# Angel3245/p2pfl

Measured on AMD Instinct MI355X. Metric: train samples/s (aggregate over peers); wall-clock per FedAvg round in ms_per_step, higher is better.
Workload: dtype bf16; 1 GPU; model=MNIST-CNN (p2pfl CNN: conv5x5 32/64 + FC 3136-2048-10, 6.5M params), Adam 1e-3, global_batch=32, per_peer_round=2700 train + 300 val + 500 test samples, 1 epoch, parallelism=gossip-p2p

## Files before the change

### csrc/cnn.h

```cpp
#pragma once
#include <hip/hip_runtime.h>
#include <stdint.h>

namespace p2cnn {

constexpr int kImg = 28;
constexpr int kC1 = 32;
constexpr int kC2 = 64;
constexpr int kFeat = 3136;
constexpr int kHid = 2048;
constexpr int kCls = 10;
constexpr int kTaps = 25;
constexpr int kXcdSplits = 7;
bool xcd_align();

struct AdamCfg {
  float lr, beta1, beta2, eps, weight_decay;
};

struct Offsets {
  int64_t c1w, c1b, c2w, c2b, l1w, l1b, l2w, l2b;
};

void conv1_fwd(const uint8_t* x, const int64_t* idx, const float* params, Offsets off, uint16_t* p1, uint8_t* am1,
// ... 7 lines not shown

void gemm_skinny(const uint16_t* A, const uint16_t* Bt, float* slabs, int mrows, int N, int K, int S, hipStream_t s);

void head(const float* slabs, int S, int mrows, const float* params, Offsets off, const int64_t* labels,
          const int64_t* idx, int B, int train, uint16_t* H, uint16_t* dH, float* dlogits, float* stats,
          const uint16_t* w2bf, hipStream_t s);

void fc1_wgrad_adam(const uint16_t* dH, const uint16_t* a1, int mrows, float* params, float* m, float* v,
                    float* gdump, uint16_t* w1bf, uint16_t* w1tbf, Offsets off, const int* adam_t, int t_off,
                    AdamCfg cfg, hipStream_t s);

void route_fc2(const uint16_t* dH, const uint16_t* w1t, const uint8_t* am2, int mrows, int B, uint16_t* dc2m,
               float* gb, const float* dlogits, const uint16_t* H, float* params, float* m, float* v, float* gdump,
               Offsets off, const int* adam_t, int t_off, AdamCfg cfg, bool with_fc2, hipStream_t s);

void route_fc2_rm(const uint16_t* dH, const uint16_t* w1, const uint8_t* am2, int mrows, int B, uint16_t* dc2m,
                  float* gb, const float* dlogits, const uint16_t* H, float* params, float* m, float* v,
                  float* gdump, Offsets off, const int* adam_t, int t_off, AdamCfg cfg, bool with_fc2,
                  float* ws, int* ctr, hipStream_t s);

void conv2_bwd(const uint16_t* dc2m, const uint16_t* p1s, const uint8_t* am1, const uint16_t* w2q, const uint8_t* x,
               const int64_t* idx, float* wslab1, float* wslab2, int B, hipStream_t s);

void conv_adam(const float* wslab1, const float* wslab2, const float* gb, int B, float* params, float* m, float* v,
               float* gdump, uint16_t* w2r, uint16_t* w2q, Offsets off, const int* adam_t, int t_off, AdamCfg cfg,
               hipStream_t s);

struct FwdNext {
  const uint8_t* x;
  const int64_t* idx;
  uint16_t* p1;
  uint8_t* am1;
  uint16_t* p1s;
  uint16_t* a1;
  uint8_t* am2;
  int B;
  int* sync;
};
void fc1_conv_adam_fwd(const uint16_t* dH, const uint16_t* a1, int mrows, const float* wslab1, const float* wslab2,
                       const float* gb, int B, float* params, float* m, float* v, float* gdump, uint16_t* w1bf,
                       uint16_t* w1tbf, uint16_t* w2r, uint16_t* w2q, Offsets off, const int* adam_t, int t_off,
                       AdamCfg cfg, const float* dlogits, const uint16_t* H, uint16_t* w2bf, const FwdNext& f,
                       hipStream_t s);

void fc1_conv_adam(const uint16_t* dH, const uint16_t* a1, int mrows, const float* wslab1, const float* wslab2,
                   const float* gb, int B, float* params, float* m, float* v, float* gdump, uint16_t* w1bf,
                   uint16_t* w1tbf, uint16_t* w2r, uint16_t* w2q, Offsets off, const int* adam_t, int t_off,
                   AdamCfg cfg, const float* dlogits, const uint16_t* H, uint16_t* w2bf, hipStream_t s);

void pack_shadows(const float* params, Offsets off, uint16_t* w2r, uint16_t* w2q, uint16_t* w1bf, uint16_t* w1tbf,
                  uint16_t* w2bf, hipStream_t s);

constexpr int kP1sPlane = 18 * 16;
constexpr int kP1s = 5 * kC1 * kP1sPlane;
constexpr int kDgTiles = 7;
constexpr int kSlab1 = kC1 * kTaps + kC1;
constexpr int kWgG = 2;
constexpr int kSlab2 = kTaps * kC2 * kC1;
__host__ __device__ inline int wgrad_groups(int B) { return (B + kWgG - 1) / kWgG; }

}
```

### csrc/cnn_bindings.cpp

```cpp
#include <torch/extension.h>
#include <c10/hip/HIPStream.h>
#include <c10/core/DeviceGuard.h>

#include "cnn.h"

namespace {

using p2cnn::AdamCfg;
using p2cnn::Offsets;

hipStream_t stream() { return c10::hip::getCurrentHIPStream().stream(); }

template <typename T>
T* ptr(const torch::Tensor& t, c10::ScalarType st, int64_t min_numel, const char* name, int align = 16) {
  TORCH_CHECK(t.defined() && t.is_cuda(), name, ": expected a GPU tensor");
  TORCH_CHECK(t.scalar_type() == st, name, ": wrong dtype ", t.scalar_type());
  TORCH_CHECK(t.is_contiguous(), name, ": must be contiguous");
  TORCH_CHECK(t.numel() >= min_numel, name, ": needs >= ", min_numel, " elements, got ", t.numel());
  TORCH_CHECK(reinterpret_cast<uintptr_t>(t.data_ptr()) % align == 0, name, ": must be ", align, "-byte aligned");
  return reinterpret_cast<T*>(t.data_ptr());
}
template <typename T>
T* optr(const c10::optional<torch::Tensor>& t, c10::ScalarType st, int64_t min_numel, const char* name,
        int align = 16) {
// ... 133 lines not shown
  const auto dHp = reinterpret_cast<uint16_t*>(ptr<at::BFloat16>(dH, torch::kBFloat16, mrows * 2048, "dH"));
  const auto w1p = reinterpret_cast<uint16_t*>(ptr<at::BFloat16>(w1, torch::kBFloat16, 2048 * 3136, "w1"));
  const auto am2p = ptr<uint8_t>(am2, torch::kUInt8, B * 3136, "am2");
  const auto dc2p = reinterpret_cast<uint16_t*>(ptr<at::BFloat16>(dc2m, torch::kBFloat16, B * 64 * 224, "dc2m"));
  const auto gbp = ptr<float>(gb, torch::kFloat32, B * 3136, "gb");
  const auto dlp = ptr<float>(dlogits, torch::kFloat32, B * 10, "dlogits");
  const auto Hp = reinterpret_cast<uint16_t*>(ptr<at::BFloat16>(H, torch::kBFloat16, B * 2048, "H"));
  float* pp = ptr<float>(params, torch::kFloat32, n, "params");
  float* mp = ptr<float>(m, torch::kFloat32, n, "m");
  float* vp = ptr<float>(v, torch::kFloat32, n, "v");
  float* gd = optr<float>(gdump, torch::kFloat32, n, "gdump");
  const int* tp = ptr<int>(adam_t, torch::kInt32, 1, "adam_t", 4);
  if (row_major) {
    float* wsp = optr<float>(ws, torch::kFloat32, 98 * 2 * mrows * 32, "ws");
    int* cp = optr<int>(ctr, torch::kInt32, 98, "ctr", 4);
    p2cnn::route_fc2_rm(dHp, w1p, am2p, int(mrows), int(B), dc2p, gbp, dlp, Hp, pp, mp, vp, gd, o, tp, int(t_off),
                        cfg(lr, b1, b2, eps, wd), with_fc2, wsp, cp, stream());
  } else {
    p2cnn::route_fc2(dHp, w1p, am2p, int(mrows), int(B), dc2p, gbp, dlp, Hp, pp, mp, vp, gd, o, tp, int(t_off),
                     cfg(lr, b1, b2, eps, wd), with_fc2, stream());
  }
}

void k_conv2_bwd(torch::Tensor dc2m, torch::Tensor p1s, torch::Tensor am1, torch::Tensor w2q, torch::Tensor x,
                 c10::optional<torch::Tensor> idx, torch::Tensor wslab1, torch::Tensor wslab2, int64_t B) {
  const c10::DeviceGuard g(dc2m.device());
  TORCH_CHECK(B >= 1 && B <= 64, "bad batch");
  TORCH_CHECK(x.numel() % 784 == 0, "x must be [N,1,28,28] uint8");
  if (!idx.has_value()) TORCH_CHECK(x.numel() / 784 >= B, "x has fewer than B rows");
  p2cnn::conv2_bwd(reinterpret_cast<uint16_t*>(ptr<at::BFloat16>(dc2m, torch::kBFloat16, B * 64 * 224, "dc2m")),
                   reinterpret_cast<uint16_t*>(ptr<at::BFloat16>(p1s, torch::kBFloat16, B * p2cnn::kP1s, "p1s")),
                   ptr<uint8_t>(am1, torch::kUInt8, B * 196 * 32, "am1"),
                   reinterpret_cast<uint16_t*>(ptr<at::BFloat16>(w2q, torch::kBFloat16, 51200, "w2q")),
                   ptr<uint8_t>(x, torch::kUInt8, 784, "x", 1), idx_ptr(idx, B),
                   ptr<float>(wslab1, torch::kFloat32, B * p2cnn::kDgTiles * p2cnn::kSlab1, "wslab1"),
                   ptr<float>(wslab2, torch::kFloat32, p2cnn::wgrad_groups(int(B)) * int64_t(p2cnn::kSlab2), "wslab2"),
                   int(B), stream());
}

void k_conv_adam(torch::Tensor wslab1, torch::Tensor wslab2, torch::Tensor gb, int64_t B, torch::Tensor params,
                 torch::Tensor m,
                 torch::Tensor v, c10::optional<torch::Tensor> gdump, torch::Tensor w2r, torch::Tensor w2q,
                 std::vector<int64_t> off, torch::Tensor adam_t, int64_t t_off, double lr, double b1, double b2,
                 double eps, double wd) {
  const c10::DeviceGuard g(params.device());
  Offsets o = offsets(off);
  const int64_t n = params_end(o);
  TORCH_CHECK(B >= 1 && B <= 64, "bad batch");
  p2cnn::conv_adam(ptr<float>(wslab1, torch::kFloat32, B * p2cnn::kDgTiles * p2cnn::kSlab1, "wslab1"),
                   ptr<float>(wslab2, torch::kFloat32, p2cnn::wgrad_groups(int(B)) * int64_t(p2cnn::kSlab2), "wslab2"),
                   ptr<float>(gb, torch::kFloat32, B * 3136, "gb"), int(B),
                   ptr<float>(params, torch::kFloat32, n, "params"), ptr<float>(m, torch::kFloat32, n, "m"),
                   ptr<float>(v, torch::kFloat32, n, "v"), optr<float>(gdump, torch::kFloat32, n, "gdump"),
                   reinterpret_cast<uint16_t*>(ptr<at::BFloat16>(w2r, torch::kBFloat16, 51200, "w2r")),
                   reinterpret_cast<uint16_t*>(ptr<at::BFloat16>(w2q, torch::kBFloat16, 51200, "w2q")), o,
                   ptr<int>(adam_t, torch::kInt32, 1, "adam_t", 4), int(t_off), cfg(lr, b1, b2, eps, wd), stream());
}

void k_fc1_conv_adam(torch::Tensor dH, torch::Tensor a1, int64_t mrows, torch::Tensor wslab1, torch::Tensor wslab2,
                     torch::Tensor gb, int64_t B, torch::Tensor params, torch::Tensor m, torch::Tensor v,
                     c10::optional<torch::Tensor> gdump, torch::Tensor w1bf, c10::optional<torch::Tensor> w1tbf, torch::Tensor w2r,
                     torch::Tensor w2q, std::vector<int64_t> off, torch::Tensor adam_t, int64_t t_off, double lr,
                     double b1, double b2, double eps, double wd, c10::optional<torch::Tensor> dlogits,
                     c10::optional<torch::Tensor> H, c10::optional<torch::Tensor> w2bf) {
  const c10::DeviceGuard g(params.device());
  check_batch(int(B), int(mrows));
  TORCH_CHECK(mrows <= 64, "fc1_conv_adam: mrows must be 32 or 64");
  TORCH_CHECK(dlogits.has_value() == H.has_value(), "fc1_conv_adam: pass both dlogits and H or neither");
  Offsets o = offsets(off);
  const int64_t n = params_end(o);
  p2cnn::fc1_conv_adam(
      reinterpret_cast<uint16_t*>(ptr<at::BFloat16>(dH, torch::kBFloat16, mrows * 2048, "dH")),
      reinterpret_cast<uint16_t*>(ptr<at::BFloat16>(a1, torch::kBFloat16, mrows * 3136, "a1")), int(mrows),
      ptr<float>(wslab1, torch::kFloat32, B * p2cnn::kDgTiles * p2cnn::kSlab1, "wslab1"),
      ptr<float>(wslab2, torch::kFloat32, p2cnn::wgrad_groups(int(B)) * int64_t(p2cnn::kSlab2), "wslab2"),
      ptr<float>(gb, torch::kFloat32, B * 3136, "gb"), int(B), ptr<float>(params, torch::kFloat32, n, "params"),
      ptr<float>(m, torch::kFloat32, n, "m"), ptr<float>(v, torch::kFloat32, n, "v"),
      optr<float>(gdump, torch::kFloat32, n, "gdump"),
      reinterpret_cast<uint16_t*>(ptr<at::BFloat16>(w1bf, torch::kBFloat16, 2048 * 3136, "w1bf")),
      reinterpret_cast<uint16_t*>(optr<at::BFloat16>(w1tbf, torch::kBFloat16, 2048 * 3136, "w1tbf")),
      reinterpret_cast<uint16_t*>(ptr<at::BFloat16>(w2r, torch::kBFloat16, 51200, "w2r")),
      reinterpret_cast<uint16_t*>(ptr<at::BFloat16>(w2q, torch::kBFloat16, 51200, "w2q")), o,
      ptr<int>(adam_t, torch::kInt32, 1, "adam_t", 4), int(t_off), cfg(lr, b1, b2, eps, wd),
      optr<float>(dlogits, torch::kFloat32, B * 10, "dlogits"),
      reinterpret_cast<const uint16_t*>(optr<at::BFloat16>(H, torch::kBFloat16, B * 2048, "H")),
      reinterpret_cast<uint16_t*>(optr<at::BFloat16>(w2bf, torch::kBFloat16, 10 * 2048, "w2bf")), stream());
}

void k_fc1_conv_adam_fwd(torch::Tensor dH, torch::Tensor a1, int64_t mrows, torch::Tensor wslab1, torch::Tensor wslab2,
                         torch::Tensor gb, int64_t B, torch::Tensor params, torch::Tensor m, torch::Tensor v,
                         c10::optional<torch::Tensor> gdump, torch::Tensor w1bf, c10::optional<torch::Tensor> w1tbf,
                         torch::Tensor w2r, torch::Tensor w2q, std::vector<int64_t> off, torch::Tensor adam_t,
                         int64_t t_off, double lr, double b1, double b2, double eps, double wd,
                         c10::optional<torch::Tensor> dlogits, c10::optional<torch::Tensor> H,
                         c10::optional<torch::Tensor> w2bf, torch::Tensor x, c10::optional<torch::Tensor> idx,
                         torch::Tensor p1, torch::Tensor am1, torch::Tensor p1s, torch::Tensor a1n, torch::Tensor am2,
                         int64_t Bn, torch::Tensor sync) {
  const c10::DeviceGuard g(params.device());
  check_batch(int(B), int(mrows));
  check_batch(int(Bn), int(mrows));
  TORCH_CHECK(mrows <= 64, "fc1_conv_adam_fwd: mrows must be 32 or 64");
  TORCH_CHECK(dlogits.has_value() == H.has_value(), "fc1_conv_adam_fwd: pass both dlogits and H or neither");
  TORCH_CHECK(x.numel() % 784 == 0, "x must be [N,1,28,28] uint8");
  if (!idx.has_value()) TORCH_CHECK(x.numel() / 784 >= Bn, "x has fewer than Bn rows");
  TORCH_CHECK(a1n.data_ptr() != a1.data_ptr(), "fc1_conv_adam_fwd: the next step's A1 must be the other buffer");
  Offsets o = offsets(off);
  const int64_t n = params_end(o);
  p2cnn::FwdNext f{};
  f.x = ptr<uint8_t>(x, torch::kUInt8, 784, "x", 1);
// ... 40 lines not shown

namespace p2cnn {
void init_attributes();
}

void register_cnn(pybind11::module& m) {
  auto c = m.def_submodule("cnn", "fused MNIST-CNN training step kernels");
  c.def("init", &p2cnn::init_attributes, "set kernel attributes (call before HIP graph capture)");
  c.def("conv1_fwd", &k_conv1_fwd);
  c.def("conv2_fwd", &k_conv2_fwd);
  c.def("conv12_fwd", &k_conv12_fwd);
  c.def("gemm_skinny", &k_gemm_skinny);
  c.def("head", &k_head, pybind11::arg("slabs"), pybind11::arg("S"), pybind11::arg("mrows"), pybind11::arg("params"),
        pybind11::arg("off"), pybind11::arg("labels"), pybind11::arg("idx"), pybind11::arg("B"), pybind11::arg("train"),
        pybind11::arg("H"), pybind11::arg("dH"), pybind11::arg("dlogits"), pybind11::arg("stats"),
        pybind11::arg("w2bf") = pybind11::none());
  c.def("route_fc2", &k_route_fc2, pybind11::arg("dH"), pybind11::arg("w1"), pybind11::arg("am2"), pybind11::arg("mrows"), pybind11::arg("B"),
        pybind11::arg("dc2m"), pybind11::arg("gb"), pybind11::arg("dlogits"), pybind11::arg("H"), pybind11::arg("params"), pybind11::arg("m"), pybind11::arg("v"),
        pybind11::arg("gdump"), pybind11::arg("off"), pybind11::arg("adam_t"), pybind11::arg("t_off"), pybind11::arg("lr"), pybind11::arg("b1"),
        pybind11::arg("b2"), pybind11::arg("eps"), pybind11::arg("wd"), pybind11::arg("with_fc2") = true, pybind11::arg("row_major") = false,
        pybind11::arg("ws") = pybind11::none(), pybind11::arg("ctr") = pybind11::none());
  c.def("fc1_wgrad_adam", &k_fc1_wgrad_adam);
  c.def("conv2_bwd", &k_conv2_bwd);
  c.def("conv_adam", &k_conv_adam);
  c.def("fc1_conv_adam", &k_fc1_conv_adam, pybind11::arg("dH"), pybind11::arg("a1"), pybind11::arg("mrows"), pybind11::arg("wslab1"),
        pybind11::arg("wslab2"), pybind11::arg("gb"), pybind11::arg("B"), pybind11::arg("params"), pybind11::arg("m"), pybind11::arg("v"), pybind11::arg("gdump"),
        pybind11::arg("w1bf"), pybind11::arg("w1tbf"), pybind11::arg("w2r"), pybind11::arg("w2q"), pybind11::arg("off"), pybind11::arg("adam_t"),
        pybind11::arg("t_off"), pybind11::arg("lr"), pybind11::arg("b1"), pybind11::arg("b2"), pybind11::arg("eps"), pybind11::arg("wd"),
        pybind11::arg("dlogits") = pybind11::none(), pybind11::arg("H") = pybind11::none(),
        pybind11::arg("w2bf") = pybind11::none());
  c.def("fc1_conv_adam_fwd", &k_fc1_conv_adam_fwd);
  c.def("pack_shadows", &k_pack_shadows, pybind11::arg("params"), pybind11::arg("off"), pybind11::arg("w2r"),
        pybind11::arg("w2q"), pybind11::arg("w1bf"), pybind11::arg("w1tbf"), pybind11::arg("w2bf") = pybind11::none());
  c.def("wgrad_groups", [](int64_t B) { return int64_t(p2cnn::wgrad_groups(int(B))); },
        "conv2 weight-gradient partial slabs (of 51200 floats) written for a batch of B");
}
```

### csrc/cnn_bwd.hip

```cpp
#include <cstdlib>

#include "cnn.h"
#include "cnn_fwd_dev.h"
#include "common.h"

namespace p2cnn {
using namespace p2;

typedef __bf16 bf16x8_t __attribute__((ext_vector_type(8)));
typedef short s16x4 __attribute__((ext_vector_type(4)));
P2_DEVICE f32x16 mfma32b(uint4 a, uint4 b, f32x16 c) {
  return __builtin_amdgcn_mfma_f32_32x32x16_bf16(__builtin_bit_cast(bf16x8_t, a), __builtin_bit_cast(bf16x8_t, b), c,
                                                  0, 0, 0);
}
P2_DEVICE int acc_row_b(int i, int h) { return (i & 3) + 8 * (i >> 2) + 4 * h; }
P2_DEVICE uint4 pack8(const uint16_t (&v)[8]) {
  uint4 q;
  q.x = uint32_t(v[0]) | (uint32_t(v[1]) << 16);
  q.y = uint32_t(v[2]) | (uint32_t(v[3]) << 16);
  q.z = uint32_t(v[4]) | (uint32_t(v[5]) << 16);
  q.w = uint32_t(v[6]) | (uint32_t(v[7]) << 16);
  return q;
}

// ... 716 lines not shown
    const int pos = tile * 32 + acc_row_b(i, h);
    const uint8_t a = acode[i];
    if (pos < 196 && a < 4) {
      const int yy = 2 * (pos / 14) + (a >> 1), xx = 2 * (pos % 14) + (a & 1);
      const float gv = acc[i];
      bs += gv;
#pragma unroll
      for (int ky = 0; ky < 5; ++ky)
#pragma unroll
        for (int kx = 0; kx < 5; ++kx) wg[ky * 5 + kx] = fmaf(gv, xs[yy + ky][xx + kx], wg[ky * 5 + kx]);
    }
  }
#pragma unroll
  for (int t = 0; t < kTaps; ++t) wg[t] += __shfl_xor(wg[t], 32, 64);
  bs += __shfl_xor(bs, 32, 64);
  if (h == 0) {
    float* o = wslab1 + (size_t(b) * kDgTiles + tile) * kSlab1;
#pragma unroll
    for (int t = 0; t < kTaps; ++t) o[r * kTaps + t] = wg[t];
    o[kC1 * kTaps + r] = bs;
  }
}

__global__ __launch_bounds__(256) void conv2_bwd_kernel(const uint16_t* __restrict__ dc2m,
                                                        const uint16_t* __restrict__ p1s,
                                                        const uint8_t* __restrict__ am1,
                                                        const uint16_t* __restrict__ w2q,
                                                        const uint8_t* __restrict__ xds,
                                                        const int64_t* __restrict__ idx, float* __restrict__ wslab1,
                                                        float* __restrict__ wslab2, int B, int first_block,
                                                        int wg_blocks, int stream_w, int wg_first) {
  extern __shared__ __attribute__((aligned(16))) char smem[];
  const int nd = 2 * B;
  int j = blockIdx.x + first_block;
  if (wg_first) j = j < int(gridDim.x) - nd ? j + nd : j - (int(gridDim.x) - nd);
  if (j < nd) {
    if (stream_w)
      conv2_dgrad_block<true>(j & 1, j >> 1, dc2m, am1, w2q, xds, idx, wslab1, smem);
    else
      conv2_dgrad_block<false>(j & 1, j >> 1, dc2m, am1, w2q, xds, idx, wslab1, smem);
  } else if (wg_blocks) {
    const int k = j - nd;
    conv2_wgrad_block(k / 5, k % 5, dc2m, p1s, wslab2, B, smem);
  } else {
    const int k = (j - nd) * 4 + (threadIdx.x >> 6);
    if (k < kTaps * wgrad_groups(B)) conv2_wgrad_role(k % kTaps, k / kTaps, dc2m, p1s, wslab2, B);
  }
}

void conv2_bwd(const uint16_t* dc2m, const uint16_t* p1s, const uint8_t* am1, const uint16_t* w2q, const uint8_t* x,
               const int64_t* idx, float* wslab1, float* wslab2, int B, hipStream_t s) {
  static const int roles = [] {
    const char* e = getenv("P2CNN_CONV2BWD_ROLES");
    return e ? atoi(e) : 3;
  }();
  static const int wg_blocks = [] {
    const char* e = getenv("P2CNN_CONV2_WG_BLOCKS");
    return e ? atoi(e) : 1;
  }();
  static const int stream_w = [] {
    const char* e = getenv("P2CNN_DGRAD_STREAM_W");
    return e ? atoi(e) : 0;
  }();
  static const int wg_first = [] {
    const char* e = getenv("P2CNN_CONV2BWD_WG_FIRST");
    return e ? atoi(e) : 0;
  }();
  const int nd = 2 * B, nw = wg_blocks ? 5 * wgrad_groups(B) : (kTaps * wgrad_groups(B) + 3) / 4;
  const int first = roles == 2 ? nd : 0;
  const int blocks = roles == 1 ? nd : roles == 2 ? nw : nd + nw;
  hipLaunchKernelGGL(conv2_bwd_kernel, dim3(blocks), dim3(256), kDgLds, s, dc2m, p1s, am1, w2q, x, idx, wslab1, wslab2,
                     B, first, wg_blocks, stream_w, roles == 3 ? wg_first : 0);
}

constexpr int kC1Blocks = kSlab1 / 16;

constexpr int kConvAdamLds = (kTaps * (kC1 + 1) + 256) * 4;

template <bool WT>
P2_DEVICE void st_p(float* p, float v) {
  if constexpr (WT)
    __hip_atomic_store(p, v, __ATOMIC_RELAXED, __HIP_MEMORY_SCOPE_AGENT);
  else
    *p = v;
}
template <bool WT>
P2_DEVICE void st_h(uint16_t* p, uint16_t v) {
  if constexpr (WT)
    __hip_atomic_store(p, v, __ATOMIC_RELAXED, __HIP_MEMORY_SCOPE_AGENT);
  else
    *p = v;
}

template <bool WT = false>
P2_DEVICE void conv_adam_body(int blk, const float* __restrict__ ws1, const float* __restrict__ ws2,
// ... 117 lines not shown
    }
  }
}

__global__ __launch_bounds__(256) void conv_adam_kernel(const float* __restrict__ ws1, const float* __restrict__ ws2,
                                                        const float* __restrict__ gb, int B, float* __restrict__ p,
                                                        float* __restrict__ m, float* __restrict__ v,
                                                        float* __restrict__ gdump, uint16_t* __restrict__ w2r,
                                                        uint16_t* __restrict__ w2q, Offsets off,
                                                        const int* __restrict__ adam_t, int t_off, AdamCfg cfg) {
  __shared__ __attribute__((aligned(16))) char smem[kConvAdamLds];
  conv_adam_body(blockIdx.x, ws1, ws2, gb, B, p, m, v, gdump, w2r, w2q, off, adam_t, t_off, cfg, smem);
}

constexpr int kFc2Blocks256 = (kCls * kHid + kCls + 255) / 256;

template <int MR>
__global__ __launch_bounds__(256) void fc1_conv_adam_kernel(
    const uint16_t* __restrict__ dH, const uint16_t* __restrict__ a1, const float* __restrict__ ws1,
    const float* __restrict__ ws2, const float* __restrict__ gb, int B, float* __restrict__ p, float* __restrict__ m,
    float* __restrict__ v, float* __restrict__ gdump, uint16_t* __restrict__ w1bf, uint16_t* __restrict__ w1tbf,
    uint16_t* __restrict__ w2r, uint16_t* __restrict__ w2q, Offsets off, const int* __restrict__ adam_t, int t_off,
    AdamCfg cfg, const float* __restrict__ dlogits, const uint16_t* __restrict__ H, int nf2,
    uint16_t* __restrict__ w2bf) {
  constexpr int kLds = Fc1Lds<MR>::kBytes > kConvAdamLds ? Fc1Lds<MR>::kBytes : kConvAdamLds;
  __shared__ __attribute__((aligned(16))) char smem[kLds];
  constexpr int kCA = kC2 + kC1Blocks, kBx = (kFeat + 127) / 128;
  int j = blockIdx.x;
  if (j < nf2) {
    fc2_role<256>(j, dlogits, H, B, p, m, v, gdump, off, adam_t, t_off, cfg, w2bf);
    return;
  }
  j -= nf2;
  if (j < kCA) {
    conv_adam_body(j, ws1, ws2, gb, B, p, m, v, gdump, w2r, w2q, off, adam_t, t_off, cfg, smem);
    return;
  }
  const int f = j - kCA;
  fc1_wgrad_adam_body<MR>(f % kBx, f / kBx, dH, a1, p, m, v, gdump, w1bf, w1tbf, off, adam_t, t_off, cfg, smem);
}

void fc1_conv_adam(const uint16_t* dH, const uint16_t* a1, int mrows, const float* wslab1, const float* wslab2,
                   const float* gb, int B, float* params, float* m, float* v, float* gdump, uint16_t* w1bf,
                   uint16_t* w1tbf, uint16_t* w2r, uint16_t* w2q, Offsets off, const int* adam_t, int t_off,
                   AdamCfg cfg, const float* dlogits, const uint16_t* H, uint16_t* w2bf, hipStream_t s) {
  const int nf2 = dlogits ? kFc2Blocks256 : 0;
  const dim3 grid(nf2 + kC2 + kC1Blocks + ((kFeat + 127) / 128) * (kHid / 32));
  if (mrows == 32)
    hipLaunchKernelGGL(fc1_conv_adam_kernel<32>, grid, dim3(256), 0, s, dH, a1, wslab1, wslab2, gb, B, params, m, v,
                       gdump, w1bf, w1tbf, w2r, w2q, off, adam_t, t_off, cfg, dlogits, H, nf2, w2bf);
  else
    hipLaunchKernelGGL(fc1_conv_adam_kernel<64>, grid, dim3(256), 0, s, dH, a1, wslab1, wslab2, gb, B, params, m, v,
                       gdump, w1bf, w1tbf, w2r, w2q, off, adam_t, t_off, cfg, dlogits, H, nf2, w2bf);
}

P2_DEVICE void wait_tickets(int* ctr, int target, int* stall) {
  if (threadIdx.x == 0) {
    int it = 0;
    while (__hip_atomic_load(ctr, __ATOMIC_RELAXED, __HIP_MEMORY_SCOPE_AGENT) < target) {
      if (++it > (1 << 22)) {
        __hip_atomic_store(stall, 1, __ATOMIC_RELAXED, __HIP_MEMORY_SCOPE_AGENT);
        break;
      }
      __builtin_amdgcn_s_sleep(2);
    }
  }
  __syncthreads();
}
P2_DEVICE void put_ticket(int* ctr) {
  asm volatile("s_waitcnt vmcnt(0)" ::: "memory");
  __syncthreads();
  if (threadIdx.x == 0) __hip_atomic_fetch_add(ctr, 1, __ATOMIC_RELAXED, __HIP_MEMORY_SCOPE_AGENT);
}

template <int MR>
__global__ __launch_bounds__(256) void fc1_conv_adam_fwd_kernel(
// ... 59 lines not shown
  const int n1 = 7 * f.B, n2 = (14 * f.B + 3) / 4;
  const dim3 grid(nf2 + kC2 + kC1Blocks + n1 + n2 + ((kFeat + 127) / 128) * (kHid / 32));
  if (mrows == 32)
    hipLaunchKernelGGL(fc1_conv_adam_fwd_kernel<32>, grid, dim3(256), 0, s, dH, a1, wslab1, wslab2, gb, B, params, m,
                       v, gdump, w1bf, w1tbf, w2r, w2q, off, adam_t, t_off, cfg, dlogits, H, nf2, w2bf, f);
  else
    hipLaunchKernelGGL(fc1_conv_adam_fwd_kernel<64>, grid, dim3(256), 0, s, dH, a1, wslab1, wslab2, gb, B, params, m,
                       v, gdump, w1bf, w1tbf, w2r, w2q, off, adam_t, t_off, cfg, dlogits, H, nf2, w2bf, f);
}

void conv_adam(const float* wslab1, const float* wslab2, const float* gb, int B, float* params, float* m, float* v,
               float* gdump, uint16_t* w2r, uint16_t* w2q, Offsets off, const int* adam_t, int t_off, AdamCfg cfg,
               hipStream_t s) {
  hipLaunchKernelGGL(conv_adam_kernel, dim3(kC2 + kC1Blocks), dim3(256), 0, s, wslab1, wslab2, gb, B, params, m, v,
                     gdump, w2r, w2q, off, adam_t, t_off, cfg);
}

void init_fwd_attributes();

void init_attributes() {
  init_fwd_attributes();
  P2_CHECK(hipFuncSetAttribute(reinterpret_cast<const void*>(conv2_bwd_kernel),
                               hipFuncAttributeMaxDynamicSharedMemorySize, kDgLds));
  P2_CHECK(hipFuncSetAttribute(reinterpret_cast<const void*>(route_rm_kernel<1, 1>),
                               hipFuncAttributeMaxDynamicSharedMemorySize, kRouteRmLds));
  P2_CHECK(hipFuncSetAttribute(reinterpret_cast<const void*>(route_rm_kernel<2, 1>),
                               hipFuncAttributeMaxDynamicSharedMemorySize, kRouteRmLds));
  P2_CHECK(hipFuncSetAttribute(reinterpret_cast<const void*>(route_rm_kernel<1, 2>),
                               hipFuncAttributeMaxDynamicSharedMemorySize, kRouteRmLds / 2));
  P2_CHECK(hipFuncSetAttribute(reinterpret_cast<const void*>(route_rm_kernel<2, 2>),
                               hipFuncAttributeMaxDynamicSharedMemorySize, kRouteRmLds / 2));
}

}
```

### p2pfl_amd/learning/fused_cnn.py

```python

from __future__ import annotations

import collections
import math
import os
import threading
import time
from typing import Any, Dict, List, Optional, Tuple

import torch

from p2pfl_amd import ops
from p2pfl_amd.learning.arena import FlatParams, ModuleArena
from p2pfl_amd.learning.host_completion import HostCompletions
from p2pfl_amd.learning.torch_learner import TorchLearner
from p2pfl_amd.management.logger import logger
from p2pfl_amd.utils.lockcheck import make_lock, make_rlock
from p2pfl_amd.utils.streams import private_stream

_CAPTURE_LOCK = make_lock("FusedCNN._CAPTURE_LOCK")
RUN_AHEAD = max(1, int(os.environ.get("P2PFL_FIT_RUN_AHEAD", "2")))

_MERGED_ADAM = os.environ.get("P2PFL_CNN_MERGED_ADAM", "1") != "0"
_ROUTE_RM = os.environ.get("P2PFL_CNN_ROUTE_RM", "1") != "0"
_ROUTE_SPLIT = os.environ.get("P2PFL_CNN_ROUTE_SPLIT", "0") == "1"
_EVAL_LOW = os.environ.get("P2PFL_EVAL_STREAM_LOW", "1") != "0"
_EVAL_SIDE = os.environ.get("P2PFL_EVAL_SIDE_STREAM", "0")
_CONV12 = os.environ.get("P2PFL_CNN_CONV12", "0") == "1"
_FWD_IN_ADAM = os.environ.get("P2PFL_CNN_FWD_IN_ADAM", "0") == "1"
_NAMES = ("conv1.weight", "conv1.bias", "conv2.weight", "conv2.bias", "l1.weight", "l1.bias", "l2.weight", "l2.bias")
FEAT, HID = 3136, 2048


class FusedCNNEngine:

    def __init__(
        self,
        model: torch.nn.Module,
        device: Optional[torch.device] = None,
        lr: float = 1e-3,
        betas: Tuple[float, float] = (0.9, 0.999),
        eps: float = 1e-8,
        weight_decay: float = 0.0,
        mrows: int = 32,
        arena: Optional[ModuleArena] = None,
        split_fc1: Optional[int] = None,
    ) -> None:
        self.C = ops.ext().cnn
        self.C.init()
        self.device = torch.device(device) if device is not None else torch.device("cuda", torch.cuda.current_device())
        model.to(self.device)
        self.arena = arena if arena is not None else ModuleArena(model, device=self.device)
        lay = self.arena.layout
        if tuple(lay.names) != _NAMES:
            raise ValueError(f"FusedCNNEngine needs the reference CNN layout {_NAMES}, got {lay.names}")
        shapes = dict(zip(lay.names, lay.shapes))
        if shapes["conv1.weight"] != (32, 1, 5, 5) or shapes["l2.weight"][1] != HID or shapes["l2.weight"][0] != 10:
            raise ValueError("unsupported CNN configuration (needs 1x28x28 input, 10 classes)")
        self.off: List[int] = [int(o) for o in lay.offsets]
        self.lr, self.betas, self.eps, self.wd = lr, betas, eps, weight_decay
        self.mrows = mrows
        self.S1 = int(split_fc1 if split_fc1 is not None else os.environ.get("P2PFL_CNN_FC1_SPLITS", "7"))
        if not 1 <= self.S1 <= 49:
            raise ValueError(f"FC1 split count {self.S1} outside [1, 49]")
        dev, bf = self.device, torch.bfloat16
        z = lambda *s, dt=torch.float32: torch.zeros(*s, dtype=dt, device=dev)
        n = self.arena.flat.numel()
        npad = (n + 3) // 4 * 4
        self._opt_state = z(2 * npad + 4)
        self.m, self.v = self._opt_state[:n], self._opt_state[npad:npad + n]
        self.adam_t = self._opt_state[2 * npad:2 * npad + 1].view(torch.int32)
        self.w2r, self.w2q = z(51200, dt=bf), z(51200, dt=bf)
        self.route_rm = _ROUTE_RM
        self.w1bf = z(HID * FEAT, dt=bf)
        self.w1tbf = None if self.route_rm else z(HID * FEAT, dt=bf)
        self.w2bf = z(10 * HID, dt=bf) if _MERGED_ADAM else None
        M = mrows
        self.p1, self.am1 = z(M * 196 * 32, dt=bf), z(M * 196 * 32, dt=torch.uint8)
        self.p1s = z(M * 5 * 32 * 18 * 16, dt=bf)
        self._a1s = (z(M * FEAT, dt=bf), z(M * FEAT, dt=bf))
        self._par = 0
        self.am2 = z(M * FEAT, dt=torch.uint8)
        self._fwd_sync = z(4, dt=torch.int32)
        self.slabs1 = z(self.S1 * M * HID)
        self.H, self.dH = z(M * HID, dt=bf), z(M * HID, dt=bf)
        self.dlogits = z(M * 10)
        self.dc2m, self.gb = z(M * 64 * 224, dt=bf), z(M * FEAT)
# ... 33 lines not shown
            pass
        elif _CONV12:
            C.conv12_fwd(x, idx, self.params, self.off, self.w2r, None, self.am1, self.p1s if train else None, self.a1,
                         self.am2, B, M)
        else:
            C.conv1_fwd(x, idx, self.params, self.off, self.p1, self.am1, self.p1s if train else None, B)
            C.conv2_fwd(self.p1, self.w2r, self.params, self.off, self.a1, self.am2, B, M)
        C.gemm_skinny(self.a1, self.w1bf, self.slabs1, M, HID, FEAT, self.S1)
        C.head(self.slabs1, self.S1, M, self.params, self.off, labels, idx, B, train, self.H, self.dH, self.dlogits, stats,
               self.w2bf)

    def train_step_async(
        self, x: torch.Tensor, labels: torch.Tensor, idx: Optional[torch.Tensor], B: int, stats: torch.Tensor, t_off: int,
        nxt: Optional[Tuple[Optional[torch.Tensor], int]] = None, fwd_done: bool = False,
    ) -> None:
        if B > self.mrows:
            raise ValueError(f"batch {B} > engine capacity {self.mrows}")
        C, M, a = self.C, self.mrows, self._adam()
        self.forward(x, labels, idx, B, stats, True, convs=not fwd_done)
        if _MERGED_ADAM:
            C.route_fc2(self.dH, self.w1_route, self.am2, M, B, self.dc2m, self.gb, self.dlogits, self.H,
                        self.params, self.m, self.v, self.gdump, self.off, self.adam_t, t_off, *a, False, self.route_rm,
                        self.route_ws, self.route_ctr)
            C.conv2_bwd(self.dc2m, self.p1s, self.am1, self.w2q, x, idx, self.wslab1, self.wslab2, B)
            if nxt is not None and M <= 64:
                idx_n, Bn = nxt
                C.fc1_conv_adam_fwd(self.dH, self.a1, M, self.wslab1, self.wslab2, self.gb, B, self.params, self.m,
                                    self.v, self.gdump, self.w1bf, self.w1tbf, self.w2r, self.w2q, self.off, self.adam_t,
                                    t_off, *a, self.dlogits, self.H, self.w2bf, x, idx_n, self.p1, self.am1, self.p1s,
                                    self._a1s[1 - self._par], self.am2, Bn, self._fwd_sync)
                self._par ^= 1
                return
            C.fc1_conv_adam(self.dH, self.a1, M, self.wslab1, self.wslab2, self.gb, B, self.params, self.m, self.v,
                            self.gdump, self.w1bf, self.w1tbf, self.w2r, self.w2q, self.off, self.adam_t, t_off, *a,
                            self.dlogits, self.H, self.w2bf)
            return
        C.route_fc2(self.dH, self.w1_route, self.am2, M, B, self.dc2m, self.gb, self.dlogits, self.H,
                    self.params, self.m, self.v, self.gdump, self.off, self.adam_t, t_off, *a, True, self.route_rm,
                    self.route_ws, self.route_ctr)
        C.fc1_wgrad_adam(self.dH, self.a1, M, self.params, self.m, self.v, self.gdump, self.w1bf, self.w1tbf, self.off, self.adam_t, t_off, *a)
        C.conv2_bwd(self.dc2m, self.p1s, self.am1, self.w2q, x, idx, self.wslab1, self.wslab2, B)
        C.conv_adam(self.wslab1, self.wslab2, self.gb, B, self.params, self.m, self.v, self.gdump, self.w2r, self.w2q, self.off, self.adam_t, t_off, *a)

    def train_step(self, x: torch.Tensor, y: torch.Tensor) -> float:
        B = int(y.shape[0])
        self.stats.zero_()
# ... 334 lines not shown
```

Measured before the change: 407,300 samples/s.

## Host first FC1 wgrad+Adam tiles inside conv2 backward launch

Adds a conv2_bwd_fc1 kernel whose extra blocks, beyond the conv2 dgrad/wgrad roles, compute the first N FC1 weight-gradient plus Adam tiles. The following fc1_conv_adam launch then starts at that tile offset. The aim is to fill idle CUs during the small conv2 backward and shorten the critical path of the merged Adam kernel. It only applies on the non-pipelined path (no next batch, forward not already done), and the slice size defaults to 384 tiles.

```diff
diff --git a/csrc/cnn.h b/csrc/cnn.h
--- a/csrc/cnn.h
+++ b/csrc/cnn.h
@@ -53,6 +53,27 @@
 void conv2_bwd(const uint16_t* dc2m, const uint16_t* p1s, const uint8_t* am1, const uint16_t* w2q, const uint8_t* x,
                const int64_t* idx, float* wslab1, float* wslab2, int B, hipStream_t s);
 
+constexpr int kFc1Tiles = ((kFeat + 127) / 128) * (kHid / 32);
+struct Fc1Args {
+  const uint16_t* dH;
+  const uint16_t* a1;
+  int mrows;
+  float* params;
+  float* m;
+  float* v;
+  float* gdump;
+  uint16_t* w1bf;
+  uint16_t* w1tbf;
+  Offsets off;
+  const int* adam_t;
+  int t_off;
+  AdamCfg cfg;
+};
+
+int conv2_bwd_fc1(const uint16_t* dc2m, const uint16_t* p1s, const uint8_t* am1, const uint16_t* w2q, const uint8_t* x,
+                  const int64_t* idx, float* wslab1, float* wslab2, int B, const Fc1Args& f, int n_tiles,
+                  hipStream_t s);
+
 void conv_adam(const float* wslab1, const float* wslab2, const float* gb, int B, float* params, float* m, float* v,
                float* gdump, uint16_t* w2r, uint16_t* w2q, Offsets off, const int* adam_t, int t_off, AdamCfg cfg,
                hipStream_t s);
@@ -77,7 +98,8 @@
 void fc1_conv_adam(const uint16_t* dH, const uint16_t* a1, int mrows, const float* wslab1, const float* wslab2,
                    const float* gb, int B, float* params, float* m, float* v, float* gdump, uint16_t* w1bf,
                    uint16_t* w1tbf, uint16_t* w2r, uint16_t* w2q, Offsets off, const int* adam_t, int t_off,
-                   AdamCfg cfg, const float* dlogits, const uint16_t* H, uint16_t* w2bf, hipStream_t s);
+                   AdamCfg cfg, const float* dlogits, const uint16_t* H, uint16_t* w2bf, int first_tile,
+                   hipStream_t s);
 
 void pack_shadows(const float* params, Offsets off, uint16_t* w2r, uint16_t* w2q, uint16_t* w1bf, uint16_t* w1tbf,
                   uint16_t* w2bf, hipStream_t s);
diff --git a/csrc/cnn_bindings.cpp b/csrc/cnn_bindings.cpp
--- a/csrc/cnn_bindings.cpp
+++ b/csrc/cnn_bindings.cpp
@@ -179,20 +179,56 @@
   }
 }
 
+int64_t conv2_bwd_impl(torch::Tensor dc2m, torch::Tensor p1s, torch::Tensor am1, torch::Tensor w2q, torch::Tensor x,
+                       c10::optional<torch::Tensor> idx, torch::Tensor wslab1, torch::Tensor wslab2, int64_t B,
+                       const p2cnn::Fc1Args& fc, int64_t n_tiles) {
+  TORCH_CHECK(B >= 1 && B <= 64, "bad batch");
+  TORCH_CHECK(x.numel() % 784 == 0, "x must be [N,1,28,28] uint8");
+  if (!idx.has_value()) TORCH_CHECK(x.numel() / 784 >= B, "x has fewer than B rows");
+  return p2cnn::conv2_bwd_fc1(
+      reinterpret_cast<uint16_t*>(ptr<at::BFloat16>(dc2m, torch::kBFloat16, B * 64 * 224, "dc2m")),
+      reinterpret_cast<uint16_t*>(ptr<at::BFloat16>(p1s, torch::kBFloat16, B * p2cnn::kP1s, "p1s")),
+      ptr<uint8_t>(am1, torch::kUInt8, B * 196 * 32, "am1"),
+      reinterpret_cast<uint16_t*>(ptr<at::BFloat16>(w2q, torch::kBFloat16, 51200, "w2q")),
+      ptr<uint8_t>(x, torch::kUInt8, 784, "x", 1), idx_ptr(idx, B),
+      ptr<float>(wslab1, torch::kFloat32, B * p2cnn::kDgTiles * p2cnn::kSlab1, "wslab1"),
+      ptr<float>(wslab2, torch::kFloat32, p2cnn::wgrad_groups(int(B)) * int64_t(p2cnn::kSlab2), "wslab2"), int(B), fc,
+      int(n_tiles), stream());
+}
+
 void k_conv2_bwd(torch::Tensor dc2m, torch::Tensor p1s, torch::Tensor am1, torch::Tensor w2q, torch::Tensor x,
                  c10::optional<torch::Tensor> idx, torch::Tensor wslab1, torch::Tensor wslab2, int64_t B) {
   const c10::DeviceGuard g(dc2m.device());
-  TORCH_CHECK(B >= 1 && B <= 64, "bad batch");
-  TORCH_CHECK(x.numel() % 784 == 0, "x must be [N,1,28,28] uint8");
-  if (!idx.has_value()) TORCH_CHECK(x.numel() / 784 >= B, "x has fewer than B rows");
-  p2cnn::conv2_bwd(reinterpret_cast<uint16_t*>(ptr<at::BFloat16>(dc2m, torch::kBFloat16, B * 64 * 224, "dc2m")),
-                   reinterpret_cast<uint16_t*>(ptr<at::BFloat16>(p1s, torch::kBFloat16, B * p2cnn::kP1s, "p1s")),
-                   ptr<uint8_t>(am1, torch::kUInt8, B * 196 * 32, "am1"),
-                   reinterpret_cast<uint16_t*>(ptr<at::BFloat16>(w2q, torch::kBFloat16, 51200, "w2q")),
-                   ptr<uint8_t>(x, torch::kUInt8, 784, "x", 1), idx_ptr(idx, B),
-                   ptr<float>(wslab1, torch::kFloat32, B * p2cnn::kDgTiles * p2cnn::kSlab1, "wslab1"),
-                   ptr<float>(wslab2, torch::kFloat32, p2cnn::wgrad_groups(int(B)) * int64_t(p2cnn::kSlab2), "wslab2"),
-                   int(B), stream());
+  conv2_bwd_impl(dc2m, p1s, am1, w2q, x, idx, wslab1, wslab2, B, p2cnn::Fc1Args{}, 0);
+}
+
+int64_t k_conv2_bwd_fc1(torch::Tensor dc2m, torch::Tensor p1s, torch::Tensor am1, torch::Tensor w2q, torch::Tensor x,
+                        c10::optional<torch::Tensor> idx, torch::Tensor wslab1, torch::Tensor wslab2, int64_t B,
+                        torch::Tensor dH, torch::Tensor a1, int64_t mrows, torch::Tensor params, torch::Tensor m,
+                        torch::Tensor v, c10::optional<torch::Tensor> gdump, torch::Tensor w1bf,
+                        c10::optional<torch::Tensor> w1tbf, std::vector<int64_t> off, torch::Tensor adam_t,
+                        int64_t t_off, double lr, double b1, double b2, double eps, double wd, int64_t n_tiles) {
+  const c10::DeviceGuard g(dc2m.device());
+  TORCH_CHECK(mrows == 32 || mrows == 64, "conv2_bwd_fc1: mrows must be 32 or 64");
+  TORCH_CHECK(n_tiles >= 0 && n_tiles <= p2cnn::kFc1Tiles, "conv2_bwd_fc1: n_tiles ", n_tiles, " outside [0, ",
+              p2cnn::kFc1Tiles, "]");
+  Offsets o = offsets(off);
+  const int64_t n = params_end(o);
+  p2cnn::Fc1Args fc{};
+  fc.dH = reinterpret_cast<uint16_t*>(ptr<at::BFloat16>(dH, torch::kBFloat16, mrows * 2048, "dH"));
+  fc.a1 = reinterpret_cast<uint16_t*>(ptr<at::BFloat16>(a1, torch::kBFloat16, mrows * 3136, "a1"));
+  fc.mrows = int(mrows);
+  fc.params = ptr<float>(params, torch::kFloat32, n, "params");
+  fc.m = ptr<float>(m, torch::kFloat32, n, "m");
+  fc.v = ptr<float>(v, torch::kFloat32, n, "v");
+  fc.gdump = optr<float>(gdump, torch::kFloat32, n, "gdump");
+  fc.w1bf = reinterpret_cast<uint16_t*>(ptr<at::BFloat16>(w1bf, torch::kBFloat16, 2048 * 3136, "w1bf"));
+  fc.w1tbf = reinterpret_cast<uint16_t*>(optr<at::BFloat16>(w1tbf, torch::kBFloat16, 2048 * 3136, "w1tbf"));
+  fc.off = o;
+  fc.adam_t = ptr<int>(adam_t, torch::kInt32, 1, "adam_t", 4);
+  fc.t_off = int(t_off);
+  fc.cfg = cfg(lr, b1, b2, eps, wd);
+  return conv2_bwd_impl(dc2m, p1s, am1, w2q, x, idx, wslab1, wslab2, B, fc, n_tiles);
 }
 
 void k_conv_adam(torch::Tensor wslab1, torch::Tensor wslab2, torch::Tensor gb, int64_t B, torch::Tensor params,
@@ -219,10 +255,12 @@
                      c10::optional<torch::Tensor> gdump, torch::Tensor w1bf, c10::optional<torch::Tensor> w1tbf, torch::Tensor w2r,
                      torch::Tensor w2q, std::vector<int64_t> off, torch::Tensor adam_t, int64_t t_off, double lr,
                      double b1, double b2, double eps, double wd, c10::optional<torch::Tensor> dlogits,
-                     c10::optional<torch::Tensor> H, c10::optional<torch::Tensor> w2bf) {
+                     c10::optional<torch::Tensor> H, c10::optional<torch::Tensor> w2bf, int64_t first_tile) {
   const c10::DeviceGuard g(params.device());
   check_batch(int(B), int(mrows));
   TORCH_CHECK(mrows <= 64, "fc1_conv_adam: mrows must be 32 or 64");
+  TORCH_CHECK(first_tile >= 0 && first_tile <= p2cnn::kFc1Tiles, "fc1_conv_adam: first_tile ", first_tile,
+              " outside [0, ", p2cnn::kFc1Tiles, "]");
   TORCH_CHECK(dlogits.has_value() == H.has_value(), "fc1_conv_adam: pass both dlogits and H or neither");
   Offsets o = offsets(off);
   const int64_t n = params_end(o);
@@ -241,7 +279,8 @@
       ptr<int>(adam_t, torch::kInt32, 1, "adam_t", 4), int(t_off), cfg(lr, b1, b2, eps, wd),
       optr<float>(dlogits, torch::kFloat32, B * 10, "dlogits"),
       reinterpret_cast<const uint16_t*>(optr<at::BFloat16>(H, torch::kBFloat16, B * 2048, "H")),
-      reinterpret_cast<uint16_t*>(optr<at::BFloat16>(w2bf, torch::kBFloat16, 10 * 2048, "w2bf")), stream());
+      reinterpret_cast<uint16_t*>(optr<at::BFloat16>(w2bf, torch::kBFloat16, 10 * 2048, "w2bf")), int(first_tile),
+      stream());
 }
 
 void k_fc1_conv_adam_fwd(torch::Tensor dH, torch::Tensor a1, int64_t mrows, torch::Tensor wslab1, torch::Tensor wslab2,
@@ -328,13 +367,15 @@
         pybind11::arg("ws") = pybind11::none(), pybind11::arg("ctr") = pybind11::none());
   c.def("fc1_wgrad_adam", &k_fc1_wgrad_adam);
   c.def("conv2_bwd", &k_conv2_bwd);
+  c.def("conv2_bwd_fc1", &k_conv2_bwd_fc1,
+        "conv2_bwd hosting the first n_tiles FC1 weight-gradient + Adam tiles; returns the tiles hosted");
   c.def("conv_adam", &k_conv_adam);
   c.def("fc1_conv_adam", &k_fc1_conv_adam, pybind11::arg("dH"), pybind11::arg("a1"), pybind11::arg("mrows"), pybind11::arg("wslab1"),
         pybind11::arg("wslab2"), pybind11::arg("gb"), pybind11::arg("B"), pybind11::arg("params"), pybind11::arg("m"), pybind11::arg("v"), pybind11::arg("gdump"),
         pybind11::arg("w1bf"), pybind11::arg("w1tbf"), pybind11::arg("w2r"), pybind11::arg("w2q"), pybind11::arg("off"), pybind11::arg("adam_t"),
         pybind11::arg("t_off"), pybind11::arg("lr"), pybind11::arg("b1"), pybind11::arg("b2"), pybind11::arg("eps"), pybind11::arg("wd"),
         pybind11::arg("dlogits") = pybind11::none(), pybind11::arg("H") = pybind11::none(),
-        pybind11::arg("w2bf") = pybind11::none());
+        pybind11::arg("w2bf") = pybind11::none(), pybind11::arg("first_tile") = 0);
   c.def("fc1_conv_adam_fwd", &k_fc1_conv_adam_fwd);
   c.def("pack_shadows", &k_pack_shadows, pybind11::arg("params"), pybind11::arg("off"), pybind11::arg("w2r"),
         pybind11::arg("w2q"), pybind11::arg("w1bf"), pybind11::arg("w1tbf"), pybind11::arg("w2bf") = pybind11::none());
diff --git a/csrc/cnn_bwd.hip b/csrc/cnn_bwd.hip
--- a/csrc/cnn_bwd.hip
+++ b/csrc/cnn_bwd.hip
@@ -762,18 +762,13 @@
   }
 }
 
-__global__ __launch_bounds__(256) void conv2_bwd_kernel(const uint16_t* __restrict__ dc2m,
-                                                        const uint16_t* __restrict__ p1s,
-                                                        const uint8_t* __restrict__ am1,
-                                                        const uint16_t* __restrict__ w2q,
-                                                        const uint8_t* __restrict__ xds,
-                                                        const int64_t* __restrict__ idx, float* __restrict__ wslab1,
-                                                        float* __restrict__ wslab2, int B, int first_block,
-                                                        int wg_blocks, int stream_w, int wg_first) {
-  extern __shared__ __attribute__((aligned(16))) char smem[];
+P2_DEVICE void conv2_bwd_roles(int j, int nconv, const uint16_t* __restrict__ dc2m, const uint16_t* __restrict__ p1s,
+                               const uint8_t* __restrict__ am1, const uint16_t* __restrict__ w2q,
+                               const uint8_t* __restrict__ xds, const int64_t* __restrict__ idx,
+                               float* __restrict__ wslab1, float* __restrict__ wslab2, int B, int wg_blocks,
+                               int stream_w, int wg_first, char* smem) {
   const int nd = 2 * B;
-  int j = blockIdx.x + first_block;
-  if (wg_first) j = j < int(gridDim.x) - nd ? j + nd : j - (int(gridDim.x) - nd);
+  if (wg_first) j = j < nconv - nd ? j + nd : j - (nconv - nd);
   if (j < nd) {
     if (stream_w)
       conv2_dgrad_block<true>(j & 1, j >> 1, dc2m, am1, w2q, xds, idx, wslab1, smem);
@@ -788,8 +783,41 @@
   }
 }
 
-void conv2_bwd(const uint16_t* dc2m, const uint16_t* p1s, const uint8_t* am1, const uint16_t* w2q, const uint8_t* x,
-               const int64_t* idx, float* wslab1, float* wslab2, int B, hipStream_t s) {
+__global__ __launch_bounds__(256) void conv2_bwd_kernel(const uint16_t* __restrict__ dc2m,
+                                                        const uint16_t* __restrict__ p1s,
+                                                        const uint8_t* __restrict__ am1,
+                                                        const uint16_t* __restrict__ w2q,
+                                                        const uint8_t* __restrict__ xds,
+                                                        const int64_t* __restrict__ idx, float* __restrict__ wslab1,
+                                                        float* __restrict__ wslab2, int B, int first_block,
+                                                        int wg_blocks, int stream_w, int wg_first) {
+  extern __shared__ __attribute__((aligned(16))) char smem[];
+  conv2_bwd_roles(blockIdx.x + first_block, gridDim.x, dc2m, p1s, am1, w2q, xds, idx, wslab1, wslab2, B, wg_blocks,
+                  stream_w, wg_first, smem);
+}
+
+template <int MR>
+__global__ __launch_bounds__(256) void conv2_bwd_fc1_kernel(
+    const uint16_t* __restrict__ dc2m, const uint16_t* __restrict__ p1s, const uint8_t* __restrict__ am1,
+    const uint16_t* __restrict__ w2q, const uint8_t* __restrict__ xds, const int64_t* __restrict__ idx,
+    float* __restrict__ wslab1, float* __restrict__ wslab2, int B, int nconv, int wg_blocks, int stream_w,
+    int wg_first, Fc1Args f) {
+  static_assert(Fc1Lds<MR>::kBytes <= kDgLds, "the launch's dynamic LDS serves the FC1 role too");
+  extern __shared__ __attribute__((aligned(16))) char smem[];
+  constexpr int kBx = (kFeat + 127) / 128;
+  const int j = blockIdx.x;
+  if (j < nconv) {
+    conv2_bwd_roles(j, nconv, dc2m, p1s, am1, w2q, xds, idx, wslab1, wslab2, B, wg_blocks, stream_w, wg_first, smem);
+    return;
+  }
+  const int t = j - nconv;
+  fc1_wgrad_adam_body<MR>(t % kBx, t / kBx, f.dH, f.a1, f.params, f.m, f.v, f.gdump, f.w1bf, f.w1tbf, f.off, f.adam_t,
+                          f.t_off, f.cfg, smem);
+}
+
+int conv2_bwd_fc1(const uint16_t* dc2m, const uint16_t* p1s, const uint8_t* am1, const uint16_t* w2q, const uint8_t* x,
+                  const int64_t* idx, float* wslab1, float* wslab2, int B, const Fc1Args& f, int n_tiles,
+                  hipStream_t s) {
   static const int roles = [] {
     const char* e = getenv("P2CNN_CONV2BWD_ROLES");
     return e ? atoi(e) : 3;
@@ -809,8 +837,22 @@
   const int nd = 2 * B, nw = wg_blocks ? 5 * wgrad_groups(B) : (kTaps * wgrad_groups(B) + 3) / 4;
   const int first = roles == 2 ? nd : 0;
   const int blocks = roles == 1 ? nd : roles == 2 ? nw : nd + nw;
-  hipLaunchKernelGGL(conv2_bwd_kernel, dim3(blocks), dim3(256), kDgLds, s, dc2m, p1s, am1, w2q, x, idx, wslab1, wslab2,
-                     B, first, wg_blocks, stream_w, roles == 3 ? wg_first : 0);
+  const int na = roles == 3 ? n_tiles : 0;
+  if (na == 0)
+    hipLaunchKernelGGL(conv2_bwd_kernel, dim3(blocks), dim3(256), kDgLds, s, dc2m, p1s, am1, w2q, x, idx, wslab1,
+                       wslab2, B, first, wg_blocks, stream_w, roles == 3 ? wg_first : 0);
+  else if (f.mrows == 32)
+    hipLaunchKernelGGL(conv2_bwd_fc1_kernel<32>, dim3(blocks + na), dim3(256), kDgLds, s, dc2m, p1s, am1, w2q, x, idx,
+                       wslab1, wslab2, B, blocks, wg_blocks, stream_w, wg_first, f);
+  else
+    hipLaunchKernelGGL(conv2_bwd_fc1_kernel<64>, dim3(blocks + na), dim3(256), kDgLds, s, dc2m, p1s, am1, w2q, x, idx,
+                       wslab1, wslab2, B, blocks, wg_blocks, stream_w, wg_first, f);
+  return na;
+}
+
+void conv2_bwd(const uint16_t* dc2m, const uint16_t* p1s, const uint8_t* am1, const uint16_t* w2q, const uint8_t* x,
+               const int64_t* idx, float* wslab1, float* wslab2, int B, hipStream_t s) {
+  conv2_bwd_fc1(dc2m, p1s, am1, w2q, x, idx, wslab1, wslab2, B, Fc1Args{}, 0, s);
 }
 
 constexpr int kC1Blocks = kSlab1 / 16;
@@ -974,7 +1016,7 @@
     float* __restrict__ v, float* __restrict__ gdump, uint16_t* __restrict__ w1bf, uint16_t* __restrict__ w1tbf,
     uint16_t* __restrict__ w2r, uint16_t* __restrict__ w2q, Offsets off, const int* __restrict__ adam_t, int t_off,
     AdamCfg cfg, const float* __restrict__ dlogits, const uint16_t* __restrict__ H, int nf2,
-    uint16_t* __restrict__ w2bf) {
+    uint16_t* __restrict__ w2bf, int f0) {
   constexpr int kLds = Fc1Lds<MR>::kBytes > kConvAdamLds ? Fc1Lds<MR>::kBytes : kConvAdamLds;
   __shared__ __attribute__((aligned(16))) char smem[kLds];
   constexpr int kCA = kC2 + kC1Blocks, kBx = (kFeat + 127) / 128;
@@ -988,22 +1030,23 @@
     conv_adam_body(j, ws1, ws2, gb, B, p, m, v, gdump, w2r, w2q, off, adam_t, t_off, cfg, smem);
     return;
   }
-  const int f = j - kCA;
+  const int f = j - kCA + f0;
   fc1_wgrad_adam_body<MR>(f % kBx, f / kBx, dH, a1, p, m, v, gdump, w1bf, w1tbf, off, adam_t, t_off, cfg, smem);
 }
 
 void fc1_conv_adam(const uint16_t* dH, const uint16_t* a1, int mrows, const float* wslab1, const float* wslab2,
                    const float* gb, int B, float* params, float* m, float* v, float* gdump, uint16_t* w1bf,
                    uint16_t* w1tbf, uint16_t* w2r, uint16_t* w2q, Offsets off, const int* adam_t, int t_off,
-                   AdamCfg cfg, const float* dlogits, const uint16_t* H, uint16_t* w2bf, hipStream_t s) {
+                   AdamCfg cfg, const float* dlogits, const uint16_t* H, uint16_t* w2bf, int first_tile,
+                   hipStream_t s) {
   const int nf2 = dlogits ? kFc2Blocks256 : 0;
-  const dim3 grid(nf2 + kC2 + kC1Blocks + ((kFeat + 127) / 128) * (kHid / 32));
+  const dim3 grid(nf2 + kC2 + kC1Blocks + kFc1Tiles - first_tile);
   if (mrows == 32)
     hipLaunchKernelGGL(fc1_conv_adam_kernel<32>, grid, dim3(256), 0, s, dH, a1, wslab1, wslab2, gb, B, params, m, v,
-                       gdump, w1bf, w1tbf, w2r, w2q, off, adam_t, t_off, cfg, dlogits, H, nf2, w2bf);
+                       gdump, w1bf, w1tbf, w2r, w2q, off, adam_t, t_off, cfg, dlogits, H, nf2, w2bf, first_tile);
   else
     hipLaunchKernelGGL(fc1_conv_adam_kernel<64>, grid, dim3(256), 0, s, dH, a1, wslab1, wslab2, gb, B, params, m, v,
-                       gdump, w1bf, w1tbf, w2r, w2q, off, adam_t, t_off, cfg, dlogits, H, nf2, w2bf);
+                       gdump, w1bf, w1tbf, w2r, w2q, off, adam_t, t_off, cfg, dlogits, H, nf2, w2bf, first_tile);
 }
 
 P2_DEVICE void wait_tickets(int* ctr, int target, int* stall) {
@@ -1109,6 +1152,10 @@
   init_fwd_attributes();
   P2_CHECK(hipFuncSetAttribute(reinterpret_cast<const void*>(conv2_bwd_kernel),
                                hipFuncAttributeMaxDynamicSharedMemorySize, kDgLds));
+  P2_CHECK(hipFuncSetAttribute(reinterpret_cast<const void*>(conv2_bwd_fc1_kernel<32>),
+                               hipFuncAttributeMaxDynamicSharedMemorySize, kDgLds));
+  P2_CHECK(hipFuncSetAttribute(reinterpret_cast<const void*>(conv2_bwd_fc1_kernel<64>),
+                               hipFuncAttributeMaxDynamicSharedMemorySize, kDgLds));
   P2_CHECK(hipFuncSetAttribute(reinterpret_cast<const void*>(route_rm_kernel<1, 1>),
                                hipFuncAttributeMaxDynamicSharedMemorySize, kRouteRmLds));
   P2_CHECK(hipFuncSetAttribute(reinterpret_cast<const void*>(route_rm_kernel<2, 1>),
diff --git a/p2pfl_amd/learning/fused_cnn.py b/p2pfl_amd/learning/fused_cnn.py
--- a/p2pfl_amd/learning/fused_cnn.py
+++ b/p2pfl_amd/learning/fused_cnn.py
@@ -28,6 +28,8 @@
 _EVAL_SIDE = os.environ.get("P2PFL_EVAL_SIDE_STREAM", "0")
 _CONV12 = os.environ.get("P2PFL_CNN_CONV12", "0") == "1"
 _FWD_IN_ADAM = os.environ.get("P2PFL_CNN_FWD_IN_ADAM", "0") == "1"
+FC1_SLICE_DEFAULT = 384
+FC1_TILES = 1600
 _NAMES = ("conv1.weight", "conv1.bias", "conv2.weight", "conv2.bias", "l1.weight", "l1.bias", "l2.weight", "l2.bias")
 FEAT, HID = 3136, 2048
 
@@ -45,6 +47,7 @@
         mrows: int = 32,
         arena: Optional[ModuleArena] = None,
         split_fc1: Optional[int] = None,
+        fc1_slice: Optional[int] = None,
     ) -> None:
         self.C = ops.ext().cnn
         self.C.init()
@@ -63,6 +66,9 @@
         self.S1 = int(split_fc1 if split_fc1 is not None else os.environ.get("P2PFL_CNN_FC1_SPLITS", "7"))
         if not 1 <= self.S1 <= 49:
             raise ValueError(f"FC1 split count {self.S1} outside [1, 49]")
+        self.fc1_slice = int(fc1_slice if fc1_slice is not None else os.environ.get("P2PFL_CNN_FC1_SLICE", FC1_SLICE_DEFAULT))
+        if not 0 <= self.fc1_slice <= FC1_TILES:
+            raise ValueError(f"FC1 slice {self.fc1_slice} outside [0, {FC1_TILES}]")
         dev, bf = self.device, torch.bfloat16
         z = lambda *s, dt=torch.float32: torch.zeros(*s, dtype=dt, device=dev)
         n = self.arena.flat.numel()
@@ -142,6 +148,14 @@
             C.route_fc2(self.dH, self.w1_route, self.am2, M, B, self.dc2m, self.gb, self.dlogits, self.H,
                         self.params, self.m, self.v, self.gdump, self.off, self.adam_t, t_off, *a, False, self.route_rm,
                         self.route_ws, self.route_ctr)
+            if nxt is None and not fwd_done and self.fc1_slice:
+                na = C.conv2_bwd_fc1(self.dc2m, self.p1s, self.am1, self.w2q, x, idx, self.wslab1, self.wslab2, B,
+                                     self.dH, self.a1, M, self.params, self.m, self.v, self.gdump, self.w1bf,
+                                     self.w1tbf, self.off, self.adam_t, t_off, *a, self.fc1_slice)
+                C.fc1_conv_adam(self.dH, self.a1, M, self.wslab1, self.wslab2, self.gb, B, self.params, self.m, self.v,
+                                self.gdump, self.w1bf, self.w1tbf, self.w2r, self.w2q, self.off, self.adam_t, t_off, *a,
+                                self.dlogits, self.H, self.w2bf, na)
+                return
             C.conv2_bwd(self.dc2m, self.p1s, self.am1, self.w2q, x, idx, self.wslab1, self.wslab2, B)
             if nxt is not None and M <= 64:
                 idx_n, Bn = nxt
```

After: 423,000 samples/s (median of 6 runs). 3.9% higher.
